# HUSRCF/JaTSR-Just-audio-transformer-super-solution

Hardware: AMD Instinct MI355X
Metric: DiT latent-frames/sec (B=28,C=1024,T=512, 50-step CFG) (higher is better)
Workload: dtype bf16; 1 GPU; v3mod2 DiT 50-step CFG=3.0 flow-matching sampling, hipGraph, B=28/GPU C=1024 T=512; B_per_gpu=28, global_batch=28, T=512, C=1024, euler_steps=50, weights=recipe (random-init, non-zero adaLN/final), parallelism=replicas x1, no collective in the loop, rccl_ranks=1

## Files before the change

jatsr-just-audio-transformer-super-solution_amd/csrc/gemm.hip:

```cpp
#include "jat_kernels.h"
#include "jat_dtype.h"

#include <type_traits>

typedef jat_opx8 bf16x8;
typedef __attribute__((ext_vector_type(4))) float f32x4;
typedef __attribute__((ext_vector_type(4))) unsigned u32x4;
typedef __attribute__((address_space(3))) void* lds_ptr_t;

template <int I, int N, class F>
__device__ __forceinline__ void static_for(F&& f) {
  if constexpr (I < N) {
    f(std::integral_constant<int, I>{});
    static_for<I + 1, N>(f);
  }
}

__device__ __forceinline__ unsigned short f2bf(float f) { return jat_f2op(f); }
__device__ __forceinline__ uint2 pack4(float a, float b, float c, float d) {
  uint2 r;
  r.x = jat_pack2(a, b);
  r.y = jat_pack2(c, d);
  return r;
}
// ... 1042 lines not shown
  const int tiles_m = p.M / BM, tiles_n = p.N / BN, ntiles = tiles_m * tiles_n;
  const int nk = p.K / 64;
  auto coords = [&](int v, int& m0, int& n0) {
    const int q = ntiles >> 3, r = ntiles & 7, xcd = v & 7;
    const int id = (xcd < r ? xcd * (q + 1) : r * (q + 1) + (xcd - r) * q) + (v >> 3);
    constexpr int GROUP = 8;
    const int per_group = GROUP * tiles_n;
    const int first_m = (id / per_group) * GROUP;
    const int gsz = min(tiles_m - first_m, GROUP);
    const int in_g = id % per_group;
    m0 = (first_m + in_g % gsz) * BM;
    n0 = (in_g / gsz) * BN;
  };
  const int srow = lane >> 3, schunk = (lane & 7) ^ srow;
  const int frow = lane & 15, fg = lane >> 4;
  const int a_row_off = (wm * TM * 16 + frow) * 128;
  const int b_row_off = (wn * TN * 16 + frow) * 128;
  const int coff0 = ((0 + fg) ^ (frow & 7)) * 16, coff1 = ((4 + fg) ^ (frow & 7)) * 16;
  unsigned oa0[CA0], oa1[CA1], ob0[CB0], ob1[CB1];
  int la0[CA0], la1[CA1], lb0[CB0], lb1[CB1];
  auto piece_row = [&](int q, int per, int tiles, int first) {
    const int w = q / per, in = q - w * per;
    return w * tiles * 16 + first * 16 + in * 8;
  };
#pragma unroll
  for (int j = 0; j < CA0; ++j) {
    const int r = piece_row(min(wave + 8 * j, PA0 - 1), TMa * 2, TM, 0);
    oa0[j] = (unsigned)((r + srow) * (int)p.lda * 2 + schunk * 16);
    la0[j] = r * 128;
  }
#pragma unroll
  for (int j = 0; j < CA1; ++j) {
    const int r = piece_row(min(wave + 8 * j, PA1 - 1), TMb * 2, TM, TMa);
    oa1[j] = (unsigned)((r + srow) * (int)p.lda * 2 + schunk * 16);
    la1[j] = r * 128;
  }
#pragma unroll
  for (int j = 0; j < CB0; ++j) {
    const int r = piece_row(min(wave + 8 * j, PB0 - 1), TNa * 2, TN, 0);
    ob0[j] = (unsigned)((r + srow) * (int)p.ldw * 2 + schunk * 16);
    lb0[j] = A_BYTES + r * 128;
  }
#pragma unroll
  for (int j = 0; j < CB1; ++j) {
    const int r = piece_row(min(wave + 8 * j, PB1 - 1), TNb * 2, TN, TNa);
    ob1[j] = (unsigned)((r + srow) * (int)p.ldw * 2 + schunk * 16);
    lb1[j] = A_BYTES + r * 128;
  }
  const char *a_base, *b_base;
  auto dma_a0 = [&](int st, int kt) {
#pragma unroll
    for (int j = 0; j < CA0; ++j)
      __builtin_amdgcn_global_load_lds((const void*)(a_base + kt * 128 + oa0[j]), (lds_ptr_t)(smem + st * STAGE + la0[j]), 16, 0, 0);
  };
  auto dma_a1 = [&](int st, int kt) {
#pragma unroll
    for (int j = 0; j < CA1; ++j)
      __builtin_amdgcn_global_load_lds((const void*)(a_base + kt * 128 + oa1[j]), (lds_ptr_t)(smem + st * STAGE + la1[j]), 16, 0, 0);
  };
  auto dma_b0 = [&](int st, int kt) {
#pragma unroll
    for (int j = 0; j < CB0; ++j)
      __builtin_amdgcn_global_load_lds((const void*)(b_base + kt * 128 + ob0[j]), (lds_ptr_t)(smem + st * STAGE + lb0[j]), 16, 0, 0);
  };
  auto dma_b1 = [&](int st, int kt) {
#pragma unroll
    for (int j = 0; j < CB1; ++j)
      __builtin_amdgcn_global_load_lds((const void*)(b_base + kt * 128 + ob1[j]), (lds_ptr_t)(smem + st * STAGE + lb1[j]), 16, 0, 0);
  };
  auto dma_tile = [&](int st, int kt) { dma_a0(st, kt); dma_b0(st, kt); dma_b1(st, kt); dma_a1(st, kt); };
  auto dma_x = [&](int m0, int n0) {
    {
      const int q = wave % XB_PIECES;
      const int foff = min(q * 256, BN - 256);
      const float* src = (p.bias ? p.bias + n0 : (const float*)p.W) + foff + lane * 4;
      __builtin_amdgcn_global_load_lds((const void*)src, (lds_ptr_t)(smem + XB_OFF + foff * 4), 16, 0, 0);
    }
#pragma unroll
    for (int j = 0; j < CXP; ++j) {
      const int q = min(wave + 8 * j, XP_PIECES - 1);
      const float* src = (p.rs_part ? p.rs_part + (int64_t)m0 * 16 : (const float*)p.A) + q * 256 + lane * 4;
      __builtin_amdgcn_global_load_lds((const void*)src, (lds_ptr_t)(smem + XP_OFF + q * 1024), 16, 0, 0);
    }
  };

  f32x4 acc[TM][TN];
  bf16x8 fa[2][TMa], fb[2][TNa];
  auto rd_a = [&](int st, int i0, int cnt) {
    const char* sA = smem + st * STAGE + a_row_off + i0 * 2048;
#pragma unroll
    for (int i = 0; i < TMa; ++i)
      if (i < cnt) {
        fa[0][i] = *(const bf16x8*)(sA + i * 2048 + coff0);
        fa[1][i] = *(const bf16x8*)(sA + i * 2048 + coff1);
      }
  };
  auto rd_b = [&](int st, int j0, int cnt) {
    const char* sB = smem + st * STAGE + A_BYTES + b_row_off + j0 * 2048;
#pragma unroll
    for (int j = 0; j < TNa; ++j)
      if (j < cnt) {
        fb[0][j] = *(const bf16x8*)(sB + j * 2048 + coff0);
        fb[1][j] = *(const bf16x8*)(sB + j * 2048 + coff1);
      }
  };
#define JAT_Q(I0, IC, J0, JC)                                                                                   \
  _Pragma("unroll") for (int ks = 0; ks < 2; ++ks)                                                              \
  _Pragma("unroll") for (int i = 0; i < (IC); ++i)                                                              \
  _Pragma("unroll") for (int j = 0; j < (JC); ++j)                                                              \
    acc[(I0) + i][(J0) + j] = JAT_MFMA_16x16x32(fb[ks][j], fa[ks][i], acc[(I0) + i][(J0) + j], 0, 0, 0);
#define JAT_LOAD_END()                              \
  asm volatile("s_waitcnt lgkmcnt(0)" ::: "memory"); \
  __builtin_amdgcn_sched_barrier(0);                \
  __builtin_amdgcn_s_barrier();                     \
  __builtin_amdgcn_s_setprio(1);
#define JAT_MMA_END()                 \
  __builtin_amdgcn_s_setprio(0);      \
  __builtin_amdgcn_sched_barrier(0);  \
  __builtin_amdgcn_s_barrier();
  auto kloop = [&]() __attribute__((always_inline)) {
#pragma unroll
    for (int i = 0; i < TM; ++i)
#pragma unroll
      for (int j = 0; j < TN; ++j) acc[i][j] = f32x4{0.f, 0.f, 0.f, 0.f};
    __builtin_amdgcn_s_barrier();
    if (grp == 1) __builtin_amdgcn_s_barrier();
    auto ktile = [&](int t, int st) __attribute__((always_inline)) {
      const bool more2 = t + 2 < nk;
      const bool more1 = t >= 1 && t + 1 < nk;
      rd_b(st, 0, TNa);
      __builtin_amdgcn_sched_barrier(0);
      rd_a(st, 0, TMa);
      if (more1) dma_b0(st ^ 1, t + 1);
      JAT_LOAD_END()
      JAT_Q(0, TMa, 0, TNa)
      JAT_MMA_END()
      rd_b(st, TNa, TNb);
      if (more2) dma_a0(st, t + 2);
      JAT_LOAD_END()
      JAT_Q(0, TMa, TNa, TNb)
      JAT_MMA_END()
      rd_a(st, TMa, TMb);
      if (more2) dma_b1(st, t + 2);
      JAT_LOAD_END()
      JAT_Q(TMa, TMb, TNa, TNb)
      JAT_MMA_END()
      rd_b(st, 0, TNa);
      if (more2) {
        dma_a1(st, t + 2);
        asm volatile("s_waitcnt vmcnt(%0)" ::"n"(CA0 + CB1 + CA1) : "memory");
      } else {
        asm volatile("s_waitcnt vmcnt(0)" ::: "memory");
      }
      JAT_LOAD_END()
      JAT_Q(TMa, TMb, 0, TNa)
      JAT_MMA_END()
    };
    for (int t = 0; t < nk; t += 2) {
      ktile(t, 0);
      if (t + 1 < nk) ktile(t + 1, 1);
    }
    if (grp == 0) __builtin_amdgcn_s_barrier();
  };
#undef JAT_Q
#undef JAT_LOAD_END
#undef JAT_MMA_END

  const float invk = 1.0f / (float)p.K;
  const unsigned sl0 = (unsigned)(uintptr_t)(lds_ptr_t)(smem + STAGE + wave * (2 * SLAB));
  const unsigned sl1 = sl0 + SLAB;
  const unsigned wslab = frow * RS + fg * 8;
  int rowt[NCH], soff[NCH], goff[NCH];
#pragma unroll
  for (int t = 0; t < NCH; ++t) {
    const int c = lane + 64 * t;
    rowt[t] = c / CPR;
    const int cc = c - rowt[t] * CPR;
    soff[t] = min(rowt[t], 15) * RS + cc * 16;
    goff[t] = rowt[t] * (int)p.ldo * 2 + cc * 16;
  }
  auto epilogue = [&](int m0, int n0, auto&& prefetch) __attribute__((always_inline)) {
    float rstd[TM];
    float4 bb[TN];
#pragma unroll
    for (int i = 0; i < TM; ++i) {
      rstd[i] = 1.0f;
      if (p.rs_part) {
        const char* rp = smem + XP_OFF + (wm * TM * 16 + i * 16 + frow) * 64;
        const float4 c0 = *(const float4*)rp, c1 = *(const float4*)(rp + 16), c2 = *(const float4*)(rp + 32), c3 = *(const float4*)(rp + 48);
        const float s0 = (c0.x + c0.y) + (c0.z + c0.w), s1 = (c1.x + c1.y) + (c1.z + c1.w);
        const float s2 = (c2.x + c2.y) + (c2.z + c2.w), s3 = (c3.x + c3.y) + (c3.z + c3.w);
        rstd[i] = rsqrtf(((s0 + s1) + (s2 + s3)) * invk + 1e-6f);
      }
    }
#pragma unroll
    for (int j = 0; j < TN; ++j)
      bb[j] = p.bias ? *(const float4*)(smem + XB_OFF + (wn * TN * 16 + j * 16 + fg * 4) * 4) : float4{0.f, 0.f, 0.f, 0.f};
    asm volatile("s_waitcnt lgkmcnt(0)" ::: "memory");
    __builtin_amdgcn_sched_barrier(0);
    __builtin_amdgcn_s_barrier();
    prefetch();
    char* const obase = (char*)p.out + ((int64_t)(m0 + wm * TM * 16) * p.ldo + n0 + wn * TN * 16) * 2;
    u32x4 raw[NCH];
    auto vwrite = [&](auto gc, auto kc) __attribute__((always_inline)) {
      constexpr int g = decltype(gc)::value, k = decltype(kc)::value;
      constexpr int NJ = (2 * k + 1 < TN) ? 2 : 1;
      f32x2 h[2 * NJ];
#pragma unroll
      for (int jj = 0; jj < NJ; ++jj) {
        const f32x4 v = acc[g][2 * k + jj] * rstd[g];
        h[2 * jj] = f32x2{v[0] + bb[2 * k + jj].x, v[1] + bb[2 * k + jj].y};
        h[2 * jj + 1] = f32x2{v[2] + bb[2 * k + jj].z, v[3] + bb[2 * k + jj].w};
      }
      if constexpr (EPI == EPI_BF16_GELU) gelu_erf_n<2 * NJ>(h);
#pragma unroll
      for (int jj = 0; jj < NJ; ++jj) {
        const uint2 pk = pack4(h[2 * jj][0], h[2 * jj][1], h[2 * jj + 1][0], h[2 * jj + 1][1]);
        const unsigned long long pk64 = (unsigned long long)pk.x | ((unsigned long long)pk.y << 32);
        const unsigned waddr = (g & 1 ? sl1 : sl0) + wslab + ((2 * k + jj) * 32);
        asm volatile("ds_write_b64 %0, %1" ::"v"(waddr), "v"(pk64) : "memory");
      }
    };
    auto sread = [&](auto gc) __attribute__((always_inline)) {
      constexpr int g = decltype(gc)::value;
      static_for<0, NCH>([&](auto tc) __attribute__((always_inline)) {
        constexpr int t = decltype(tc)::value;
        const unsigned raddr = (g & 1 ? sl1 : sl0) + soff[t];
        u32x4 r;
        asm volatile("ds_read_b128 %0, %1" : "=v"(r) : "v"(raddr) : "memory");
        raw[t] = r;
      });
    };
    auto swait = [&]() __attribute__((always_inline)) {
      asm volatile("s_waitcnt lgkmcnt(0)" ::: "memory");
      static_for<0, NCH>([&](auto tc) __attribute__((always_inline)) {
        u32x4 r = raw[decltype(tc)::value];
        asm volatile("" : "+v"(r));
        raw[decltype(tc)::value] = r;
      });
    };
    auto gstore = [&](auto gc, auto tc) __attribute__((always_inline)) {
      constexpr int g = decltype(gc)::value, t = decltype(tc)::value;
      if (rowt[t] < 16) *(u32x4*)(obase + (int64_t)g * 16 * p.ldo * 2 + goff[t]) = raw[t];
    };
    constexpr int NK2 = (TN + 1) / 2;
    static_assert(NK2 >= NCH, "one store slot per vector-work step");
    static_for<0, NK2>([&](auto kc) __attribute__((always_inline)) { vwrite(std::integral_constant<int, 0>{}, kc); });
    static_for<1, TM>([&](auto gc) __attribute__((always_inline)) {
      constexpr int g = decltype(gc)::value;
      sread(std::integral_constant<int, g - 1>{});
      static_for<0, NK2>([&](auto kc) __attribute__((always_inline)) {
        constexpr int k = decltype(kc)::value;
        __builtin_amdgcn_sched_barrier(0);
        vwrite(gc, kc);
        __builtin_amdgcn_sched_barrier(0);
        if constexpr (k == 0) swait();
        if constexpr (k < NCH) gstore(std::integral_constant<int, g - 1>{}, kc);
      });
      __builtin_amdgcn_sched_barrier(0);
    });
    sread(std::integral_constant<int, TM - 1>{});
    swait();
    static_for<0, NCH>([&](auto tc) __attribute__((always_inline)) { gstore(std::integral_constant<int, TM - 1>{}, tc); });
  };

  const int v0 = blockIdx.x, v1 = blockIdx.x + gridDim.x;
  const bool two = v1 < ntiles;
  int m0, n0, m1 = 0, n1 = 0;
  coords(v0, m0, n0);
  if (two) coords(v1, m1, n1);
  a_base = (const char*)(p.A + (int64_t)m0 * p.lda);
  b_base = (const char*)(p.W + (int64_t)n0 * p.ldw);
  dma_x(m0, n0);
  dma_tile(0, 0);
  if (nk > 1) {
    dma_tile(1, 1);
    asm volatile("s_waitcnt vmcnt(%0)" ::"n"(CTILE) : "memory");
  } else {
    asm volatile("s_waitcnt vmcnt(0)" ::: "memory");
  }
  kloop();
  epilogue(m0, n0, [&]() __attribute__((always_inline)) {
    if (two) {
      a_base = (const char*)(p.A + (int64_t)m1 * p.lda);
      b_base = (const char*)(p.W + (int64_t)n1 * p.ldw);
      dma_x(m1, n1);
      dma_tile(0, 0);
    }
  });
  if (!two) return;
  asm volatile("s_waitcnt lgkmcnt(0)" ::: "memory");
  __builtin_amdgcn_sched_barrier(0);
  __builtin_amdgcn_s_barrier();
  if (nk > 1) {
    dma_tile(1, 1);
    asm volatile("s_waitcnt vmcnt(%0)" ::"n"(NST + CTILE) : "memory");
  } else {
    asm volatile("s_waitcnt vmcnt(%0)" ::"n"(NST) : "memory");
  }
  kloop();
  epilogue(m1, n1, [&]() __attribute__((always_inline)) {});
}

template <int EPI, int LONGK, bool PART = false>
__global__ void __launch_bounds__(512, 1) gemm_kpair_kernel(const GemmArgs p) {
  constexpr int TM = 7, TN = 5, BM = 224, BN = 160, NW = 8;
  constexpr int A_BYTES = BM * 128, B_BYTES = BN * 128, STAGE = A_BYTES + B_BYTES;
  constexpr int PIECES = (BM + BN) / 8, CP = PIECES / NW;
  static_assert(PIECES % NW == 0, "every wave issues the same number of DMA pieces");
  static_assert(EPI == EPI_RESID || EPI == EPI_F32, "split-residual producer epilogues");
  extern __shared__ __attribute__((aligned(16))) char smem[];
#ifdef JAT_TIMELINE
  unsigned long long tl_[7] = {0, 0, 0, 0, 0, 0, 0}, tlx_[8] = {0, 0, 0, 0, 0, 0, 0, 0};
#endif
  JAT_TL(0) JAT_TLR(5)
  const int tid = threadIdx.x, lane = tid & 63;
  const int wave = __builtin_amdgcn_readfirstlane(tid >> 6);
  const int grp = wave >> 2, wq = wave & 3, wm = wq >> 1, wn = wq & 1;
  const int frow = lane & 15, fg = lane >> 4;
  const int tiles_m = p.M / BM, tiles_n = p.N / BN;
  int m0, n0;
  {
    const int nwg = gridDim.x, bid = blockIdx.x;
    const int q = nwg >> 3, r = nwg & 7, xcd = bid & 7;
    const int id = (xcd < r ? xcd * (q + 1) : r * (q + 1) + (xcd - r) * q) + (bid >> 3);
    constexpr int GROUP = 8;
    const int per_group = GROUP * tiles_n;
    const int first_m = (id / per_group) * GROUP;
    const int gsz = min(tiles_m - first_m, GROUP);
    const int in_g = id % per_group;
    m0 = (first_m + in_g % gsz) * BM;
    n0 = (in_g / gsz) * BN;
  }
  const int nk = p.K / 64;
  const int64_t kz = PART ? (int64_t)blockIdx.y * p.K : 0;
  const int srow = lane >> 3, schunk = (lane & 7) ^ srow;
  const char* psrc[CP];
  int pdst[CP];
#pragma unroll
  for (int j = 0; j < CP; ++j) {
    const int q = wave + NW * j, r = q * 8;
    pdst[j] = r * 128;
    psrc[j] = r < BM ? (const char*)(p.A + (int64_t)(m0 + r + srow) * p.lda + kz) + schunk * 16
                     : (const char*)(p.W + (int64_t)(n0 + r - BM + srow) * p.ldw + kz) + schunk * 16;
  }
  auto dma_tile = [&](int kt) {
    char* st = smem + (kt % 3) * STAGE;
#pragma unroll
    for (int j = 0; j < CP; ++j)
      __builtin_amdgcn_global_load_lds((const void*)(psrc[j] + kt * 128), (lds_ptr_t)(st + pdst[j]), 16, 0, 0);
  };
  f32x4 acc[TM][TN];
#pragma unroll
  for (int i = 0; i < TM; ++i)
#pragma unroll
    for (int j = 0; j < TN; ++j) acc[i][j] = f32x4{0.f, 0.f, 0.f, 0.f};
  bf16x8 fa[TM], fb[TN];
  const int a_off = (wm * TM * 16 + frow) * 128 + ((4 * grp + fg) ^ (frow & 7)) * 16;
  const int b_off = A_BYTES + (wn * TN * 16 + frow) * 128 + ((4 * grp + fg) ^ (frow & 7)) * 16;
  auto rd = [&](int kt) {
    const char* st = smem + (kt % 3) * STAGE;
#pragma unroll
    for (int j = 0; j < TN; ++j) fb[j] = *(const bf16x8*)(st + b_off + j * 2048);
#pragma unroll
    for (int i = 0; i < TM; ++i) fa[i] = *(const bf16x8*)(st + a_off + i * 2048);
  };
  dma_tile(0);
  if (nk > 1) dma_tile(1);
  if (nk > 2) dma_tile(2);
  if (nk > 2) asm volatile("s_waitcnt vmcnt(%0)" ::"n"(2 * CP) : "memory");
  else if (nk > 1) asm volatile("s_waitcnt vmcnt(%0)" ::"n"(CP) : "memory");
  else asm volatile("s_waitcnt vmcnt(0)" ::: "memory");
  __builtin_amdgcn_s_barrier();
  if (grp == 1) __builtin_amdgcn_s_barrier();
  JAT_TL(1)
  for (int kt = 0; kt < nk; ++kt) {
    rd(kt);
    if (kt >= 1 && kt + 2 < nk) dma_tile(kt + 2);
    if (kt + 1 < nk) {
      if (kt >= 1 && kt + 2 < nk) asm volatile("s_waitcnt vmcnt(%0)" ::"n"(CP) : "memory");
      else if (kt == 0 && nk > 2) asm volatile("s_waitcnt vmcnt(%0)" ::"n"(CP) : "memory");
      else asm volatile("s_waitcnt vmcnt(0)" ::: "memory");
    }
    asm volatile("s_waitcnt lgkmcnt(0)" ::: "memory");
    __builtin_amdgcn_sched_barrier(0);
    __builtin_amdgcn_s_barrier();
    __builtin_amdgcn_s_setprio(1);
#pragma unroll
    for (int i = 0; i < TM; ++i)
#pragma unroll
      for (int j = 0; j < TN; ++j) acc[i][j] = JAT_MFMA_16x16x32(fb[j], fa[i], acc[i][j], 0, 0, 0);
    __builtin_amdgcn_s_setprio(0);
    __builtin_amdgcn_sched_barrier(0);
    __builtin_amdgcn_s_barrier();
  }
  JAT_TL(2)
  if (grp == 0) __builtin_amdgcn_s_barrier();
  constexpr int XA = 20 * 1024, XB = 15 * 1024;
  char* xa = smem + wq * (XA + XB);
  char* xb = xa + XA;
  static_assert(4 * (XA + XB) <= 3 * STAGE, "exchange buffers fit the stages");
  if (grp == 1) {
#pragma unroll
    for (int i = 0; i < 4; ++i)
#pragma unroll
      for (int j = 0; j < TN; ++j) *(f32x4*)(xa + ((i * TN + j) * 64 + lane) * 16) = acc[i][j];
  } else {
#pragma unroll
    for (int i = 4; i < TM; ++i)
#pragma unroll
      for (int j = 0; j < TN; ++j) *(f32x4*)(xb + (((i - 4) * TN + j) * 64 + lane) * 16) = acc[i][j];
  }
  asm volatile("s_waitcnt lgkmcnt(0)" ::: "memory");
  __builtin_amdgcn_s_barrier();
  if (grp == 0) {
#pragma unroll
    for (int i = 0; i < 4; ++i)
#pragma unroll
      for (int j = 0; j < TN; ++j) acc[i][j] += *(const f32x4*)(xa + ((i * TN + j) * 64 + lane) * 16);
  } else {
#pragma unroll
    for (int i = 4; i < TM; ++i)
#pragma unroll
      for (int j = 0; j < TN; ++j) acc[i][j] += *(const f32x4*)(xb + (((i - 4) * TN + j) * 64 + lane) * 16);
  }
  asm volatile("s_waitcnt lgkmcnt(0)" ::: "memory");
  __builtin_amdgcn_s_barrier();
  JAT_TL(3)
  constexpr int RS = TN * 64 + 16, CPR8 = TN * 2, NCH8 = TN;
  static_assert(NW * 32 * RS <= 3 * STAGE, "epilogue slabs fit the stages");
  char* wbuf = smem + wave * (32 * RS);
  const int nw0 = n0 + wn * TN * 16;
  float4 bb[TN];
#pragma unroll
  for (int j = 0; j < TN; ++j) bb[j] = (!PART && p.bias) ? *(const float4*)(p.bias + nw0 + j * 16 + fg * 4) : float4{0.f, 0.f, 0.f, 0.f};
  auto up = [](unsigned u, float& a, float& b) { a = jat_lo2f(u); b = jat_hi2f(u); };
  [[maybe_unused]] float* const pout = PART ? (float*)p.out + (int64_t)blockIdx.y * p.split_stride : nullptr;
  auto half_epilogue = [&](auto i0c, auto ntc) __attribute__((always_inline)) {
    constexpr int I0 = decltype(i0c)::value, NT = decltype(ntc)::value, NG = (NT + 1) / 2;
    const int mw0 = m0 + wm * TM * 16 + I0 * 16;
    [[maybe_unused]] uint4 hi[NCH8], lo[NCH8];
    [[maybe_unused]] float4 g0[NCH8], g1[NCH8];
    auto load_chunk = [&](int ig, int t) __attribute__((always_inline)) {
      const int grows = (2 * ig + 1 < NT) ? 32 : 16;
      const int c = lane + 64 * t, row = min(c / CPR8, grows - 1), cc = c - (c / CPR8) * CPR8;
      const int m = mw0 + ig * 32 + row, n = nw0 + cc * 8;
      const unsigned off = (unsigned)(m * (int)p.ldo + n) * 2u;
      hi[t] = *(const uint4*)((const char*)p.fold_out + off);
      lo[t] = *(const uint4*)((const char*)p.fold_lo + off);
      const float* gp = p.gate + (int64_t)(m / p.ntok) * p.gate_bstride + n;
      g0[t] = *(const float4*)gp;
      g1[t] = *(const float4*)(gp + 4);
    };
    if constexpr (EPI == EPI_RESID) {
#pragma unroll
      for (int t = 0; t < NCH8; ++t) load_chunk(0, t);
    }
#pragma unroll
    for (int ig = 0; ig < NG; ++ig) {
      const int grows = (2 * ig + 1 < NT) ? 32 : 16;
#pragma unroll
      for (int ii = 0; ii < 2; ++ii)
#pragma unroll
        for (int j = 0; j < TN; ++j) if (2 * ig + ii < NT) {
          const f32x4 v = acc[I0 + (2 * ig + ii < NT ? 2 * ig + ii : 0)][j];
          *(float4*)(wbuf + (ii * 16 + frow) * RS + (j * 16 + fg * 4) * 4) =
              float4{v[0] + bb[j].x, v[1] + bb[j].y, v[2] + bb[j].z, v[3] + bb[j].w};
        }
      asm volatile("s_waitcnt lgkmcnt(0)" ::: "memory");
#pragma unroll
      for (int t = 0; t < NCH8; ++t) {
        const int c = lane + 64 * t, row = c / CPR8, cc = c - row * CPR8;
        const int m = mw0 + ig * 32 + row, n = nw0 + cc * 8;
        char* slot = wbuf + (row < 32 ? row : 0) * RS + cc * 32;
        const float4 a0 = *(const float4*)slot, a1 = *(const float4*)(slot + 16);
        float x[8] = {a0.x, a0.y, a0.z, a0.w, a1.x, a1.y, a1.z, a1.w};
        if constexpr (PART) {
          if (row < grows) {
            float* o = pout + (int64_t)m * p.ldo + n;
            *(float4*)o = a0;
            *(float4*)(o + 4) = a1;
          }
          continue;
        }
        if constexpr (EPI == EPI_RESID) {
          const unsigned hw[4] = {hi[t].x, hi[t].y, hi[t].z, hi[t].w}, lw[4] = {lo[t].x, lo[t].y, lo[t].z, lo[t].w};
          const float gg[8] = {g0[t].x, g0[t].y, g0[t].z, g0[t].w, g1[t].x, g1[t].y, g1[t].z, g1[t].w};
#pragma unroll
          for (int e = 0; e < 4; ++e) {
            float h0, h1, l0, l1;
            up(hw[e], h0, h1);
            up(lw[e], l0, l1);
            x[2 * e] = __builtin_fmaf(gg[2 * e], x[2 * e], h0 + l0);
            x[2 * e + 1] = __builtin_fmaf(gg[2 * e + 1], x[2 * e + 1], h1 + l1);
          }
          if (ig + 1 < NG) load_chunk(ig + 1, t);
        }
        unsigned ho[4], lw2[4];
        float sq = 0.f;
#pragma unroll
        for (int e = 0; e < 4; ++e) {
          const unsigned short ha = f2bf(x[2 * e]), hb = f2bf(x[2 * e + 1]);
          ho[e] = (unsigned)ha | ((unsigned)hb << 16);
          const float ra = x[2 * e] - jat_op2f(ha), rb = x[2 * e + 1] - jat_op2f(hb);
          lw2[e] = jat_pack2(ra, rb);
          const bool fuse_even = EPI != EPI_RESID || ig == 0;
          sq += fuse_even ? __builtin_fmaf(x[2 * e], x[2 * e], x[2 * e + 1] * x[2 * e + 1])
                          : __builtin_fmaf(x[2 * e + 1], x[2 * e + 1], x[2 * e] * x[2 * e]);
        }
        const bool live = row < grows;
        if (live) {
          const unsigned off = (unsigned)(m * (int)p.ldo + n) * 2u;
          *(uint4*)((char*)p.fold_out + off) = uint4{ho[0], ho[1], ho[2], ho[3]};
          *(uint4*)((char*)p.fold_lo + off) = uint4{lw2[0], lw2[1], lw2[2], lw2[3]};
        }
        if (row < 32) *(float*)slot = live ? sq : 0.f;
      }
      asm volatile("s_waitcnt lgkmcnt(0)" ::: "memory");
      if constexpr (!PART) {
        constexpr int HALF = CPR8 / 2;
        const int r = lane >> 1, h = lane & 1;
        float sq = 0.f;
#pragma unroll
        for (int cc = 0; cc < HALF; ++cc) sq += *(const float*)(wbuf + r * RS + (h * HALF + cc) * 32);
        sq += __shfl_xor(sq, 1);
        const int m = mw0 + ig * 32 + r;
        if (h == 0 && r < grows) p.fold_part[(int64_t)m * p.fold_np + nw0 / (TN * 16)] = sq;
      }
      asm volatile("s_waitcnt lgkmcnt(0)" ::: "memory");
    }
  };
  if (grp == 0) half_epilogue(std::integral_constant<int, 0>{}, std::integral_constant<int, 4>{});
  else half_epilogue(std::integral_constant<int, 4>{}, std::integral_constant<int, 3>{});
  JAT_TL_FLUSH()
}

static bool gemm_kpair_eligible(const GemmArgs& a, int epi) {
  return (epi == EPI_RESID || epi == EPI_F32) && a.fold_out && a.fold_lo && a.fold_part && a.M > 0 && a.M % 224 == 0 &&
         a.N % 160 == 0 && a.K % 64 == 0 && a.ksplit <= 1 && !a.rs_part &&
         (int64_t)a.M * a.ldo * 2 < (1ll << 32);
}
static bool gemm_kpair_part_eligible(const GemmArgs& a, int epi) {
  return epi == EPI_F32 && a.ksplit > 1 && !a.fold_out && !a.rs_part && !a.dual_rows && a.out && a.M > 0 && a.M % 224 == 0 &&
         a.N % 160 == 0 && a.K % 64 == 0 && a.K >= 192;
}
template <int EPI, int LONGK, bool PART = false>
static hipError_t launch_kpair(const GemmArgs& a, hipStream_t s) {
  constexpr int LDS = 3 * (224 + 160) * 128;
  static_assert(LDS <= 160 * 1024, "three stages must fit the 160 KiB LDS");
  static bool attr_set = false;
  auto kern = gemm_kpair_kernel<EPI, LONGK, PART>;
  if (!attr_set) {
    hipError_t e = hipFuncSetAttribute((const void*)kern, hipFuncAttributeMaxDynamicSharedMemorySize, LDS);
    if (e != hipSuccess) return e;
    attr_set = true;
  }
  hipLaunchKernelGGL(kern, dim3((a.M / 224) * (a.N / 160), PART ? a.ksplit : 1), dim3(512), LDS, s, a);
  return hipGetLastError();
}

static bool gemm_persist_eligible(const GemmArgs& a, int epi) {
  return (epi == EPI_BF16 || epi == EPI_BF16_GELU) && a.M > 0 && a.M % 224 == 0 && a.N % 320 == 0 && a.K % 64 == 0 && a.ksplit <= 1 &&
         a.dual_rows == 0 && !a.fold_out && (!a.rs_part || a.rs_np == 16) && a.ldo * 2 * 16 < (1ll << 31);
}
template <int EPI>
static hipError_t launch_persist(const GemmArgs& a, hipStream_t s) {
  constexpr int BM = 224, BN = 320, STAGE = (BM + BN) * 128;
  constexpr int LDS = 2 * STAGE + 2048 + BM * 64;
  static_assert(LDS <= 160 * 1024, "stages + bias slice + row partials must fit the 160 KiB LDS");
  static bool attr_set = false;
  auto kern = gemm_persist_kernel<2, 4, 7, 5, EPI>;
  if (!attr_set) {
    hipError_t e = hipFuncSetAttribute((const void*)kern, hipFuncAttributeMaxDynamicSharedMemorySize, LDS);
    if (e != hipSuccess) return e;
    attr_set = true;
  }
  const int tiles = (a.M / BM) * (a.N / BN);
  int grid = tiles <= 256 ? tiles : (tiles + 1) / 2;
  if (grid < 256 && tiles > 256) grid = 256;
  static const int half_env = getenv("JAT_PERSIST_HALF") ? atoi(getenv("JAT_PERSIST_HALF")) : 0;
  if (half_env > 0 && tiles > half_env && tiles <= 2 * half_env) grid = (tiles + 1) / 2;
  hipLaunchKernelGGL(kern, dim3(grid), dim3(512), LDS, s, a);
  return hipGetLastError();
}

template <int WM, int WN, int TM, int TN, int PIPE, int CE, int EPI>
static hipError_t launch_one(const GemmArgs& a, hipStream_t s) {
  constexpr int BM = WM * TM * 16, BN = WN * TN * 16;
  constexpr int LDS = (PIPE == 6 ? 3 : 2) * (BM + BN) * 128;
  static_assert(LDS <= 160 * 1024, "tile does not fit the 160 KiB LDS");
  static bool attr_set = false;
  auto kern = gemm_bf16_kernel<WM, WN, TM, TN, PIPE, CE, EPI>;
  if (!attr_set) {
    hipError_t e = hipFuncSetAttribute((const void*)kern, hipFuncAttributeMaxDynamicSharedMemorySize, LDS);
    if (e != hipSuccess) return e;
    attr_set = true;
  }
  if (a.N % BN != 0 || a.K % 64 != 0 || a.M <= 0) return hipErrorInvalidValue;
  const int tiles = ((a.M + BM - 1) / BM) * (a.N / BN);
  if (a.ksplit > 1 && EPI != EPI_F32) return hipErrorInvalidValue;
  hipLaunchKernelGGL(kern, dim3(tiles, a.ksplit > 1 ? a.ksplit : 1), dim3((WM * WN + (PIPE == 6 ? 4 : 0)) * 64), LDS, s, a);
  return hipGetLastError();
}

template <int WM, int WN, int TM, int TN, int PIPE, int CE = 0>
static hipError_t launch_epi(const GemmArgs& a, int epi, hipStream_t s) {
  switch (epi) {
    case EPI_F32: return launch_one<WM, WN, TM, TN, PIPE, CE, EPI_F32>(a, s);
    case EPI_BF16: return launch_one<WM, WN, TM, TN, PIPE, CE, EPI_BF16>(a, s);
    case EPI_BF16_GELU: return launch_one<WM, WN, TM, TN, PIPE, CE, EPI_BF16_GELU>(a, s);
    case EPI_RESID: return launch_one<WM, WN, TM, TN, PIPE, CE, EPI_RESID>(a, s);
    case EPI_QKV_ROPE: return launch_one<WM, WN, TM, TN, PIPE, CE, EPI_QKV_ROPE>(a, s);
    case EPI_UNPATCH: return launch_one<WM, WN, TM, TN, PIPE, CE, EPI_UNPATCH>(a, s);
  }
  return hipErrorInvalidValue;
}

static const int kVariantTile[][2] = {
    {0, 0}, {0, 0}, {0, 0}, {0, 0}, {0, 0}, {0, 0}, {0, 0}, {0, 0}, {0, 0}, {0, 0},
    {128, 64},
    {0, 0}, {0, 0}, {0, 0}, {0, 0}, {0, 0}, {0, 0}, {0, 0},
    {128, 160}, {0, 0}, {128, 128}, {256, 256},
    {0, 0}, {0, 0}, {0, 0},
    {256, 160}, {256, 128},
    {64, 160}, {64, 128},
    {0, 0}, {0, 0},
    {224, 320}, {256, 160}, {256, 256}, {128, 448},
    {224, 256},
    {224, 320},
    {0, 0},
    {224, 320},
    {256, 160},
};
static const int kVariantWaveN[] = {0, 0, 0, 0, 0, 0, 0, 0, 0, 0, 32, 0, 0, 0, 0, 0, 0, 0,
                                    80, 0, 64, 64, 0, 0, 0, 80, 64, 80, 64, 0, 0, 80, 80, 64, 112, 64, 80, 0, 80, 80};
int gemm_variant_wave_n(int variant) { return kVariantWaveN[variant]; }
bool gemm_variant_coalesced(int variant) { return variant >= 18; }
int gemm_num_variants() { return (int)(sizeof(kVariantTile) / sizeof(kVariantTile[0])); }

hipError_t launch_qkv_attn(const GemmArgs& a, hipStream_t s) {
  if (a.ntok != 128 || a.N % 448 != 0 || a.M % 128 != 0) return hipErrorInvalidValue;
  return launch_one<2, 4, 4, 7, 8, 0, EPI_QKV_ATTN>(a, s);
}
void gemm_variant_tile(int variant, int* bm, int* bn) {
  *bm = kVariantTile[variant][0];
  *bn = kVariantTile[variant][1];
}

bool gemm_variant_exists(int variant) {
  return variant >= 0 && variant < gemm_num_variants() && kVariantTile[variant][0] != 0;
}

hipError_t launch_gemm(const GemmArgs& a, int epi, int variant, hipStream_t s) {
  if (!gemm_variant_exists(variant)) return hipErrorInvalidValue;
  if (a.N % kVariantTile[variant][1] != 0) variant = (a.N % 128 == 0) ? 20 : 10;
  switch (variant) {
    case 10: return launch_epi<2, 2, 4, 2, 1>(a, epi, s);
    case 18: return launch_epi<2, 2, 4, 5, 2, 1>(a, epi, s);
    case 20: return launch_epi<2, 2, 4, 4, 2, 1>(a, epi, s);
    case 21: return launch_epi<2, 4, 8, 4, 2, 1>(a, epi, s);
    case 25: return launch_epi<4, 2, 4, 5, 6, 1>(a, epi, s);
    case 26: return launch_epi<4, 2, 4, 4, 6, 1>(a, epi, s);
    case 27: return launch_epi<2, 2, 2, 5, 2, 1>(a, epi, s);
    case 28: return launch_epi<2, 2, 2, 4, 2, 1>(a, epi, s);
    case 31: return launch_epi<2, 4, 7, 5, 8, 1>(a, epi, s);
    case 39:
      if (gemm_kpair_part_eligible(a, epi)) return launch_kpair<EPI_F32, 0, true>(a, s);
      if (gemm_kpair_eligible(a, epi))
        return epi != EPI_RESID ? launch_kpair<EPI_F32, 0>(a, s) : a.K >= 4096 ? launch_kpair<EPI_RESID, 1>(a, s) : launch_kpair<EPI_RESID, 0>(a, s);
      [[fallthrough]];
    case 32: return launch_epi<4, 2, 4, 5, 8, 1>(a, epi, s);
    case 33: return launch_epi<2, 4, 8, 4, 8, 1>(a, epi, s);
    case 34: return launch_epi<2, 4, 4, 7, 8, 1>(a, epi, s);
    case 35: return launch_epi<2, 4, 7, 4, 8, 1>(a, epi, s);
    case 38:
      if (gemm_persist_eligible(a, epi)) return epi == EPI_BF16 ? launch_persist<EPI_BF16>(a, s) : launch_persist<EPI_BF16_GELU>(a, s);
      [[fallthrough]];
    case 36: return launch_epi<2, 4, 7, 5, 8, 2>(a, epi, s);
  }
  return hipErrorInvalidValue;
}
```

Baseline: 40690 latent-frames/s.

## Restructure kpair epilogue: remap row groups, prefetch residual planes, add gate-stride-zero variant

Measured after the change: 41010 latent-frames/s (median of 6 runs). Within noise of the previous version (+0.8%).

```diff
diff --git a/jatsr-just-audio-transformer-super-solution_amd/csrc/gemm.hip b/jatsr-just-audio-transformer-super-solution_amd/csrc/gemm.hip
--- a/jatsr-just-audio-transformer-super-solution_amd/csrc/gemm.hip
+++ b/jatsr-just-audio-transformer-super-solution_amd/csrc/gemm.hip
@@ -1368,7 +1368,7 @@
   epilogue(m1, n1, [&]() __attribute__((always_inline)) {});
 }
 
-template <int EPI, int LONGK, bool PART = false>
+template <int EPI, int LONGK, bool PART = false, bool GS = false>
 __global__ void __launch_bounds__(512, 1) gemm_kpair_kernel(const GemmArgs p) {
   constexpr int TM = 7, TN = 5, BM = 224, BN = 160, NW = 8;
   constexpr int A_BYTES = BM * 128, B_BYTES = BN * 128, STAGE = A_BYTES + B_BYTES;
@@ -1423,13 +1423,14 @@
     for (int j = 0; j < TN; ++j) acc[i][j] = f32x4{0.f, 0.f, 0.f, 0.f};
   bf16x8 fa[TM], fb[TN];
   const int a_off = (wm * TM * 16 + frow) * 128 + ((4 * grp + fg) ^ (frow & 7)) * 16;
+  const int a_off_lo = a_off + (grp ? 4 * 2048 : 0), a_off_hi = a_off + (grp ? 0 : 3 * 2048);
   const int b_off = A_BYTES + (wn * TN * 16 + frow) * 128 + ((4 * grp + fg) ^ (frow & 7)) * 16;
   auto rd = [&](int kt) {
     const char* st = smem + (kt % 3) * STAGE;
 #pragma unroll
     for (int j = 0; j < TN; ++j) fb[j] = *(const bf16x8*)(st + b_off + j * 2048);
 #pragma unroll
-    for (int i = 0; i < TM; ++i) fa[i] = *(const bf16x8*)(st + a_off + i * 2048);
+    for (int i = 0; i < TM; ++i) fa[i] = *(const bf16x8*)(st + (i < 3 ? a_off_lo + i * 2048 : a_off_hi + (i - 3) * 2048));
   };
   dma_tile(0);
   if (nk > 1) dma_tile(1);
@@ -1462,142 +1463,177 @@
   }
   JAT_TL(2)
   if (grp == 0) __builtin_amdgcn_s_barrier();
+  int lx = lane;
+  asm volatile("" : "+v"(lx));
+  constexpr int CPR8 = TN * 2, NCH8 = TN;
+  const int nw0 = n0 + wn * TN * 16;
+  const int mw0 = m0 + wm * TM * 16 + grp * 64;
+  [[maybe_unused]] uint4 hi[NCH8], lo[NCH8];
+  [[maybe_unused]] float4 g0[NCH8], g1[NCH8];
+  auto load_planes = [&](int ln, int mg0, int grows, int t) __attribute__((always_inline)) {
+    const int c = ln + 64 * t, row = min(c / CPR8, grows - 1), cc = c - (c / CPR8) * CPR8;
+    const unsigned off = (unsigned)((mg0 + row) * (int)p.ldo + nw0 + cc * 8) * 2u;
+    hi[t] = *(const uint4*)((const char*)p.fold_out + off);
+    lo[t] = *(const uint4*)((const char*)p.fold_lo + off);
+  };
+  float4 bb[TN];
+#pragma unroll
+  for (int j = 0; j < TN; ++j) bb[j] = float4{0.f, 0.f, 0.f, 0.f};
+  if (!PART && p.bias) {
+#pragma unroll
+    for (int j = 0; j < TN; ++j) bb[j] = *(const float4*)(p.bias + nw0 + j * 16 + (lx >> 4) * 4);
+  }
+  if constexpr (EPI == EPI_RESID) {
+#pragma unroll
+    for (int t = 0; t < NCH8; ++t) load_planes(lx, mw0, 32, t);
+  }
   constexpr int XA = 20 * 1024, XB = 15 * 1024;
   char* xa = smem + wq * (XA + XB);
   char* xb = xa + XA;
   static_assert(4 * (XA + XB) <= 3 * STAGE, "exchange buffers fit the stages");
-  if (grp == 1) {
-#pragma unroll
-    for (int i = 0; i < 4; ++i)
-#pragma unroll
-      for (int j = 0; j < TN; ++j) *(f32x4*)(xa + ((i * TN + j) * 64 + lane) * 16) = acc[i][j];
-  } else {
+  {
+    char* xg = (grp ? xa + TN * 1024 : xb) + lx * 16;
+    if (grp == 1) {
+#pragma unroll
+      for (int j = 0; j < TN; ++j) *(f32x4*)(xa + lx * 16 + j * 1024) = acc[3][j];
+    }
 #pragma unroll
     for (int i = 4; i < TM; ++i)
 #pragma unroll
-      for (int j = 0; j < TN; ++j) *(f32x4*)(xb + (((i - 4) * TN + j) * 64 + lane) * 16) = acc[i][j];
+      for (int j = 0; j < TN; ++j) *(f32x4*)(xg + ((i - 4) * TN + j) * 1024) = acc[i][j];
   }
   asm volatile("s_waitcnt lgkmcnt(0)" ::: "memory");
   __builtin_amdgcn_s_barrier();
-  if (grp == 0) {
-#pragma unroll
-    for (int i = 0; i < 4; ++i)
-#pragma unroll
-      for (int j = 0; j < TN; ++j) acc[i][j] += *(const f32x4*)(xa + ((i * TN + j) * 64 + lane) * 16);
-  } else {
-#pragma unroll
-    for (int i = 4; i < TM; ++i)
-#pragma unroll
-      for (int j = 0; j < TN; ++j) acc[i][j] += *(const f32x4*)(xb + (((i - 4) * TN + j) * 64 + lane) * 16);
+  auto load_gate = [&](int ln, int mg0, int grows, int t) __attribute__((always_inline)) {
+    const int c = ln + 64 * t, row = min(c / CPR8, grows - 1), cc = c - (c / CPR8) * CPR8;
+    const float* gp = p.gate + (GS ? 0 : (int64_t)((mg0 + row) / p.ntok) * p.gate_bstride) + nw0 + cc * 8;
+    g0[t] = *(const float4*)gp;
+    g1[t] = *(const float4*)(gp + 4);
+  };
+  if constexpr (EPI == EPI_RESID) {
+#pragma unroll
+    for (int t = 0; t < NCH8; ++t) load_gate(lx, mw0, 32, t);
+  }
+  {
+    const char* xs = (grp ? xb : xa) + lx * 16;
+#pragma unroll
+    for (int i = 0; i < 3; ++i)
+#pragma unroll
+      for (int j = 0; j < TN; ++j) acc[i][j] += *(const f32x4*)(xs + (i * TN + j) * 1024);
+    if (grp == 0) {
+#pragma unroll
+      for (int j = 0; j < TN; ++j) acc[3][j] += *(const f32x4*)(xs + (3 * TN + j) * 1024);
+    }
   }
   asm volatile("s_waitcnt lgkmcnt(0)" ::: "memory");
   __builtin_amdgcn_s_barrier();
   JAT_TL(3)
-  constexpr int RS = TN * 64 + 16, CPR8 = TN * 2, NCH8 = TN;
+#pragma unroll
+  for (int i = 0; i < 4; ++i)
+#pragma unroll
+    for (int j = 0; j < TN; ++j) acc[i][j] += f32x4{bb[j].x, bb[j].y, bb[j].z, bb[j].w};
+  int le = lane;
+  asm volatile("" : "+v"(le));
+  constexpr int RS = TN * 64 + 16;
   static_assert(NW * 32 * RS <= 3 * STAGE, "epilogue slabs fit the stages");
   char* wbuf = smem + wave * (32 * RS);
-  const int nw0 = n0 + wn * TN * 16;
-  float4 bb[TN];
-#pragma unroll
-  for (int j = 0; j < TN; ++j) bb[j] = (!PART && p.bias) ? *(const float4*)(p.bias + nw0 + j * 16 + fg * 4) : float4{0.f, 0.f, 0.f, 0.f};
   auto up = [](unsigned u, float& a, float& b) { a = jat_lo2f(u); b = jat_hi2f(u); };
   [[maybe_unused]] float* const pout = PART ? (float*)p.out + (int64_t)blockIdx.y * p.split_stride : nullptr;
-  auto half_epilogue = [&](auto i0c, auto ntc) __attribute__((always_inline)) {
-    constexpr int I0 = decltype(i0c)::value, NT = decltype(ntc)::value, NG = (NT + 1) / 2;
-    const int mw0 = m0 + wm * TM * 16 + I0 * 16;
-    [[maybe_unused]] uint4 hi[NCH8], lo[NCH8];
-    [[maybe_unused]] float4 g0[NCH8], g1[NCH8];
-    auto load_chunk = [&](int ig, int t) __attribute__((always_inline)) {
-      const int grows = (2 * ig + 1 < NT) ? 32 : 16;
-      const int c = lane + 64 * t, row = min(c / CPR8, grows - 1), cc = c - (c / CPR8) * CPR8;
+  constexpr int NG = 2;
+  [[maybe_unused]] uint4 hi2[NCH8], lo2[NCH8];
+#pragma unroll
+  for (int ig = 0; ig < NG; ++ig) {
+    const int grows = (ig == 0 || grp == 0) ? 32 : 16;
+#pragma unroll
+    for (int ii = 0; ii < 2; ++ii) {
+      if (2 * ig + ii < 3 || grp == 0) {
+#pragma unroll
+        for (int j = 0; j < TN; ++j) {
+          const f32x4 v = acc[2 * ig + ii][j];
+          *(float4*)(wbuf + (ii * 16 + (le & 15)) * RS + (j * 16 + (le >> 4) * 4) * 4) = float4{v[0], v[1], v[2], v[3]};
+        }
+      }
+    }
+    if constexpr (EPI == EPI_RESID && GS) if (ig == 0) {
+      asm volatile("" ::: "memory");
+      const int gnext = grp == 0 ? 32 : 16;
+#pragma unroll
+      for (int t = 0; t < NCH8; ++t) {
+        const int c = le + 64 * t, row = min(c / CPR8, gnext - 1), cc = c - (c / CPR8) * CPR8;
+        const unsigned off = (unsigned)((mw0 + 32 + row) * (int)p.ldo + nw0 + cc * 8) * 2u;
+        hi2[t] = *(const uint4*)((const char*)p.fold_out + off);
+        lo2[t] = *(const uint4*)((const char*)p.fold_lo + off);
+      }
+    }
+    asm volatile("s_waitcnt lgkmcnt(0)" ::: "memory");
+#pragma unroll
+    for (int t = 0; t < NCH8; ++t) {
+      const int c = le + 64 * t, row = c / CPR8, cc = c - row * CPR8;
       const int m = mw0 + ig * 32 + row, n = nw0 + cc * 8;
-      const unsigned off = (unsigned)(m * (int)p.ldo + n) * 2u;
-      hi[t] = *(const uint4*)((const char*)p.fold_out + off);
-      lo[t] = *(const uint4*)((const char*)p.fold_lo + off);
-      const float* gp = p.gate + (int64_t)(m / p.ntok) * p.gate_bstride + n;
-      g0[t] = *(const float4*)gp;
-      g1[t] = *(const float4*)(gp + 4);
-    };
-    if constexpr (EPI == EPI_RESID) {
-#pragma unroll
-      for (int t = 0; t < NCH8; ++t) load_chunk(0, t);
-    }
-#pragma unroll
-    for (int ig = 0; ig < NG; ++ig) {
-      const int grows = (2 * ig + 1 < NT) ? 32 : 16;
-#pragma unroll
-      for (int ii = 0; ii < 2; ++ii)
-#pragma unroll
-        for (int j = 0; j < TN; ++j) if (2 * ig + ii < NT) {
-          const f32x4 v = acc[I0 + (2 * ig + ii < NT ? 2 * ig + ii : 0)][j];
-          *(float4*)(wbuf + (ii * 16 + frow) * RS + (j * 16 + fg * 4) * 4) =
-              float4{v[0] + bb[j].x, v[1] + bb[j].y, v[2] + bb[j].z, v[3] + bb[j].w};
-        }
-      asm volatile("s_waitcnt lgkmcnt(0)" ::: "memory");
-#pragma unroll
-      for (int t = 0; t < NCH8; ++t) {
-        const int c = lane + 64 * t, row = c / CPR8, cc = c - row * CPR8;
-        const int m = mw0 + ig * 32 + row, n = nw0 + cc * 8;
-        char* slot = wbuf + (row < 32 ? row : 0) * RS + cc * 32;
-        const float4 a0 = *(const float4*)slot, a1 = *(const float4*)(slot + 16);
-        float x[8] = {a0.x, a0.y, a0.z, a0.w, a1.x, a1.y, a1.z, a1.w};
-        if constexpr (PART) {
-          if (row < grows) {
-            float* o = pout + (int64_t)m * p.ldo + n;
-            *(float4*)o = a0;
-            *(float4*)(o + 4) = a1;
+      char* slot = wbuf + (row < 32 ? row : 0) * RS + cc * 32;
+      const float4 a0 = *(const float4*)slot, a1 = *(const float4*)(slot + 16);
+      float x[8] = {a0.x, a0.y, a0.z, a0.w, a1.x, a1.y, a1.z, a1.w};
+      if constexpr (PART) {
+        if (row < grows) {
+          float* o = pout + (int64_t)m * p.ldo + n;
+          *(float4*)o = a0;
+          *(float4*)(o + 4) = a1;
+        }
+        continue;
+      }
+      if constexpr (EPI == EPI_RESID) {
+        const uint4 hv = (GS && ig == 1) ? hi2[t] : hi[t], lv = (GS && ig == 1) ? lo2[t] : lo[t];
+        const unsigned hw[4] = {hv.x, hv.y, hv.z, hv.w}, lw[4] = {lv.x, lv.y, lv.z, lv.w};
+        const float gg[8] = {g0[t].x, g0[t].y, g0[t].z, g0[t].w, g1[t].x, g1[t].y, g1[t].z, g1[t].w};
+#pragma unroll
+        for (int e = 0; e < 4; ++e) {
+          float h0, h1, l0, l1;
+          up(hw[e], h0, h1);
+          up(lw[e], l0, l1);
+          x[2 * e] = __builtin_fmaf(gg[2 * e], x[2 * e], h0 + l0);
+          x[2 * e + 1] = __builtin_fmaf(gg[2 * e + 1], x[2 * e + 1], h1 + l1);
+        }
+        if constexpr (!GS) {
+          if (ig + 1 < NG) {
+            const int gnext = grp == 0 ? 32 : 16;
+            load_planes(le, mw0 + (ig + 1) * 32, gnext, t);
+            load_gate(le, mw0 + (ig + 1) * 32, gnext, t);
           }
-          continue;
-        }
-        if constexpr (EPI == EPI_RESID) {
-          const unsigned hw[4] = {hi[t].x, hi[t].y, hi[t].z, hi[t].w}, lw[4] = {lo[t].x, lo[t].y, lo[t].z, lo[t].w};
-          const float gg[8] = {g0[t].x, g0[t].y, g0[t].z, g0[t].w, g1[t].x, g1[t].y, g1[t].z, g1[t].w};
-#pragma unroll
-          for (int e = 0; e < 4; ++e) {
-            float h0, h1, l0, l1;
-            up(hw[e], h0, h1);
-            up(lw[e], l0, l1);
-            x[2 * e] = __builtin_fmaf(gg[2 * e], x[2 * e], h0 + l0);
-            x[2 * e + 1] = __builtin_fmaf(gg[2 * e + 1], x[2 * e + 1], h1 + l1);
-          }
-          if (ig + 1 < NG) load_chunk(ig + 1, t);
-        }
-        unsigned ho[4], lw2[4];
-        float sq = 0.f;
-#pragma unroll
-        for (int e = 0; e < 4; ++e) {
-          const unsigned short ha = f2bf(x[2 * e]), hb = f2bf(x[2 * e + 1]);
-          ho[e] = (unsigned)ha | ((unsigned)hb << 16);
-          const float ra = x[2 * e] - jat_op2f(ha), rb = x[2 * e + 1] - jat_op2f(hb);
-          lw2[e] = jat_pack2(ra, rb);
-          const bool fuse_even = EPI != EPI_RESID || ig == 0;
-          sq += fuse_even ? __builtin_fmaf(x[2 * e], x[2 * e], x[2 * e + 1] * x[2 * e + 1])
-                          : __builtin_fmaf(x[2 * e + 1], x[2 * e + 1], x[2 * e] * x[2 * e]);
-        }
-        const bool live = row < grows;
-        if (live) {
-          const unsigned off = (unsigned)(m * (int)p.ldo + n) * 2u;
-          *(uint4*)((char*)p.fold_out + off) = uint4{ho[0], ho[1], ho[2], ho[3]};
-          *(uint4*)((char*)p.fold_lo + off) = uint4{lw2[0], lw2[1], lw2[2], lw2[3]};
-        }
-        if (row < 32) *(float*)slot = live ? sq : 0.f;
-      }
-      asm volatile("s_waitcnt lgkmcnt(0)" ::: "memory");
-      if constexpr (!PART) {
-        constexpr int HALF = CPR8 / 2;
-        const int r = lane >> 1, h = lane & 1;
-        float sq = 0.f;
-#pragma unroll
-        for (int cc = 0; cc < HALF; ++cc) sq += *(const float*)(wbuf + r * RS + (h * HALF + cc) * 32);
-        sq += __shfl_xor(sq, 1);
-        const int m = mw0 + ig * 32 + r;
-        if (h == 0 && r < grows) p.fold_part[(int64_t)m * p.fold_np + nw0 / (TN * 16)] = sq;
-      }
-      asm volatile("s_waitcnt lgkmcnt(0)" ::: "memory");
-    }
-  };
-  if (grp == 0) half_epilogue(std::integral_constant<int, 0>{}, std::integral_constant<int, 4>{});
-  else half_epilogue(std::integral_constant<int, 4>{}, std::integral_constant<int, 3>{});
+        }
+      }
+      unsigned ho[4], lw2[4];
+      float sq = 0.f;
+#pragma unroll
+      for (int e = 0; e < 4; ++e) {
+        const unsigned short ha = f2bf(x[2 * e]), hb = f2bf(x[2 * e + 1]);
+        ho[e] = (unsigned)ha | ((unsigned)hb << 16);
+        const float ra = x[2 * e] - jat_op2f(ha), rb = x[2 * e + 1] - jat_op2f(hb);
+        lw2[e] = jat_pack2(ra, rb);
+        const bool fuse_even = EPI != EPI_RESID || ig == 0;
+        sq += fuse_even ? __builtin_fmaf(x[2 * e], x[2 * e], x[2 * e + 1] * x[2 * e + 1])
+                        : __builtin_fmaf(x[2 * e + 1], x[2 * e + 1], x[2 * e] * x[2 * e]);
+      }
+      const bool live = ig == 0 || row < grows;
+      if (live) {
+        const unsigned off = (unsigned)(m * (int)p.ldo + n) * 2u;
+        *(uint4*)((char*)p.fold_out + off) = uint4{ho[0], ho[1], ho[2], ho[3]};
+        *(uint4*)((char*)p.fold_lo + off) = uint4{lw2[0], lw2[1], lw2[2], lw2[3]};
+      }
+      if (row < 32) *(float*)slot = live ? sq : 0.f;
+    }
+    asm volatile("s_waitcnt lgkmcnt(0)" ::: "memory");
+    if constexpr (!PART) {
+      constexpr int HALF = CPR8 / 2;
+      const int r = le >> 1, h = le & 1;
+      float sq = 0.f;
+#pragma unroll
+      for (int cc = 0; cc < HALF; ++cc) sq += *(const float*)(wbuf + r * RS + (h * HALF + cc) * 32);
+      sq += __shfl_xor(sq, 1);
+      const int m = mw0 + ig * 32 + r;
+      if (h == 0 && r < grows) p.fold_part[(int64_t)m * p.fold_np + nw0 / (TN * 16)] = sq;
+    }
+    asm volatile("s_waitcnt lgkmcnt(0)" ::: "memory");
+  }
   JAT_TL_FLUSH()
 }
 
@@ -1610,12 +1646,14 @@
   return epi == EPI_F32 && a.ksplit > 1 && !a.fold_out && !a.rs_part && !a.dual_rows && a.out && a.M > 0 && a.M % 224 == 0 &&
          a.N % 160 == 0 && a.K % 64 == 0 && a.K >= 192;
 }
-template <int EPI, int LONGK, bool PART = false>
+template <int EPI, int LONGK, bool PART = false, bool GS = false>
 static hipError_t launch_kpair(const GemmArgs& a, hipStream_t s) {
+  if constexpr (EPI == EPI_RESID && !GS)
+    if (a.gate_bstride == 0) return launch_kpair<EPI, LONGK, PART, true>(a, s);
   constexpr int LDS = 3 * (224 + 160) * 128;
   static_assert(LDS <= 160 * 1024, "three stages must fit the 160 KiB LDS");
   static bool attr_set = false;
-  auto kern = gemm_kpair_kernel<EPI, LONGK, PART>;
+  auto kern = gemm_kpair_kernel<EPI, LONGK, PART, GS>;
   if (!attr_set) {
     hipError_t e = hipFuncSetAttribute((const void*)kern, hipFuncAttributeMaxDynamicSharedMemorySize, LDS);
     if (e != hipSuccess) return e;
```
